# BenCooper305/RL-Cattle-Herding

Hardware: AMD Instinct MI355X
Metric: env-steps/sec (agent-steps/sec) at 4096 envs/GPU, 1/2/4/8 MI355X (higher is better)
Workload: dtype f64; 1 GPU; BASELINE configs[3]: 4096 envs/GPU x (4 drones, 16 cattle), CTDE obs (12,86), random-action rollout with auto-reset; envs_per_gpu=4096, num_drones=4, num_cattle=16, mode=ctde, physics=pyb, parallelism=env-sharded x1 (no per-step collective)

## Files before the change

### rl-cattle-herding_amd/csrc/ch_step_body.h

```cpp
#pragma once
#include <hip/hip_runtime.h>

#include <atomic>

#include "ch_common.h"
#include "ch_device.h"
#include "ch_internal.h"

namespace ch {

enum { I_N = 0, I_SC, I_SCA, I_HASPREV, I_LEVEL, I_TALLY, I_SPAWN, I_ACTIVE, I_EPISODE, I_FLOCK, I_RESET, I_NEWN,
       I_HERD, I_OBSD, I_COUNT };
static_assert(I_COUNT == kV2EnvInts, "LDS env-int rows");
enum { F_D = 0, F_T, F_H, F_A, F_E, F_R, F_X0, F_X1, F_X2,
       C_PAIRS, C_ROWS, C_COWS, C_FLOCK, C_DELTA, F_W, F_Q,
       Q_LEN, C_QUEUE, F_C,
       C_EULER,
       V_DSIMD,
       F_RSV0, F_RSV1, F_RSV2,
       F_HC,
       FLAG_COUNT };
static_assert(FLAG_COUNT <= kV2Flags, "LDS flag words");
#define FL_LIST (I_COUNT * G)
#define RS_LIST (I_COUNT * G + G)
// ... 60 lines not shown
__device__ __forceinline__ void lds_wait(int* f, int target, int* err) {
    int spins = 0;
    while (__hip_atomic_load(f, __ATOMIC_RELAXED, __HIP_MEMORY_SCOPE_WORKGROUP) < target && ++spins < (1 << 22))
        __builtin_amdgcn_s_sleep(1);
    if (spins >= (1 << 22)) handoff_failed(err);
    spin_note(spins);
    __builtin_amdgcn_fence(__ATOMIC_ACQUIRE, "workgroup", "local");
}

__device__ __forceinline__ int grab(int* ctr, int n, bool skip = false) {
    if (skip) return 1 << 28;
    int b = 0;
    if ((threadIdx.x & 63) == 0) b = atomicAdd(ctr, n);
    return __builtin_amdgcn_readfirstlane(b);
}

__device__ __forceinline__ void cow_sync(int* f, int waves, bool global, int* err) {
    if (global) __builtin_amdgcn_fence(__ATOMIC_RELEASE, "workgroup");
    lds_signal(f);
    lds_wait(f, waves, err);
    if (global) __builtin_amdgcn_fence(__ATOMIC_ACQUIRE, "workgroup");
}

#define TS(slot, val) do { if (p.tstamp) p.tstamp[(long long)blockIdx.x * 128 + (slot)] = (val); } while (0)
#define CHUNK_T0 const long long ck0_ = p.tstamp ? (long long)clock64() : 0
#define TS_MAX(slot) do { if (p.tstamp && (threadIdx.x & 63) == 0) atomicMax(reinterpret_cast<unsigned long long*>(p.tstamp + (long long)blockIdx.x * 128 + (slot)), (unsigned long long)clock64()); } while (0)
#define CHUNK_T1(loop) do { if (p.tstamp && (threadIdx.x & 63) == 0 && (threadIdx.x >> 6) <= 6) { long long* q_ = p.tstamp + (long long)blockIdx.x * 128 + 64 + 10 * ((threadIdx.x >> 6) - 1) + 2 * (loop); q_[0] += 1; q_[1] += (long long)clock64() - ck0_; } } while (0)

template <class R>
struct V2Smem {
    R *cx, *cy, *cvx, *cvy, *aux, *auy;
    R *spx, *spy;
    R *dx, *dy, *dz;
    R *pa, *pb, *sa, *sb, *ca, *cb, *scat, *psp;
    R* mrew;
    R *mq, *meor;
    R* dq;
    R *rdx, *rdy, *rdz;
    R* dcow;
    R *prev, *clock, *hcx, *hcy;
    double *dxd, *dyd, *cxd, *cyd, *hcxd, *hcyd, *prevd;
    R *tgx, *tgy, *tcx, *tcy;
    R* td;
    int* cnt;
    double* met;
    int* ei;
    int* flags;
    Level* LT;
    const uint16_t* pl;
    uint8_t *dflags, *herded, *md1, *md2;
// ... 453 lines not shown
    if (nv) { nv[u] = vx; nv[GM + u] = vy; return; }
    const long long ci = (long long)e0 * M + u;
    CH_STS(&p.cattle[2 * CS + ci], vx); CH_STS(&p.cattle[3 * CS + ci], vy);
}

template <class R>
__device__ __forceinline__ void flock_combine(const StepParams<R>& p, V2Smem<R>& S, int N, int M, int e0, int u, int n,
                                              const R* td, const uint8_t* tdf, int ib, int T) {
    const R C2B = R(2 * 4.47213595499958);
    R ddx = 0, ddy = 0, sx = 0, sy = 0, gx = 0, gy = 0, cxx = 0, cyy = 0;
    int nb = 0;
    CH_UNROLL for (int k = 0; k < N; ++k) {
        if (k >= n) break;
        const int i = ib + k;
        const int f = tdf[i];
        if (f & 1) { ++nb; gx += td[i]; gy += td[T + i]; cxx += td[2 * T + i]; cyy += td[3 * T + i]; }
        if (f & 2) { sx += td[4 * T + i]; sy += td[5 * T + i]; }
    }
    if (nb > 0) { ddx = C2B * gx + C2B * cxx; ddy = C2B * gy + C2B * cyy; }
    ddx += sx; ddy += sy;
    velocity_update(p, S, M, e0, u, ddx, ddy);
}

template <class R, int MODE, int GT, int NT, int MT, bool PHYS, bool PW, bool TOBS>
__device__ __forceinline__ void step2_body(const StepParams<R>& p, int salt = 0) {
    extern __shared__ __align__(16) unsigned char smem_[];
    unsigned char* const smem = smem_ + salt;
    constexpr bool marl = MODE == 1;
    constexpr bool MIX = sizeof(R) == 4;
    using PT = double;
    constexpr bool QUAD = !marl && GT == 16 && NT == 4;
    const int G = GT ? GT : p.G, N = NT ? NT : p.NC, M = MT ? MT : p.M, P = MT ? MT * (MT - 1) / 2 : p.P;
    const int rows = marl ? N : 12;
    const V2Layout L(G, N, M, P, MODE, (int)sizeof(R), PW ? (int)(blockDim.x >> 6) - 1 : 0, !PW && p.sep);
    const bool sep = L.sep;
    V2Smem<R> S(smem, L);
    const int BS = blockDim.x + salt, tid = threadIdx.x + salt;
    const int e0 = (blockIdx.x + salt) * G;
    const int Gv = min(G, p.E - e0);
    const long long E = p.E, DS = E * N, CS = E * M;
    const int m_obs = M < 16 ? M : 16, cat_off = marl ? 18 : 34, RW = rows * 86;
    const bool task = !(p.phase_mask & 4);
    const int W1 = (BS >> 6) - 1;
    const int ct = tid - 64, CW = BS - 64;
    int* ei = S.ei;
    int* fl = S.flags;
    const Level* LT = S.LT;
    if (tid == 0) { TS(0, (long long)wall_clock64()); TS(2, (long long)clock64()); TS(12, (long long)__smid()); }
    if ((tid & 63) == 0 && tid < 256) TS(22 + (tid >> 6), (long long)__builtin_amdgcn_s_getreg((31 << 11) | 4));

    const int nd = Gv * N;
    const bool dlane = tid < nd;
    const int dg = dlane ? tid / N : 0, dk = tid - dg * N;
    const long long di = (long long)e0 * N + tid;
    R pos[3], q[4], v[3], w[3], pid[9], ql[4], rpy_in[3] = {0, 0, 0};
    R ph_lr[4] = {0, 0, 0, 0}, ph_rr[3] = {0, 0, 0};
    int stepi = 0, n0 = 0, act0 = 0, stepi_env = 0;
    double ev_acc = 0;
    R spx_r[3] = {0, 0, 0}, spy_r[3] = {0, 0, 0};
    bool co_simd = false;
    uint8_t stale_d = 1;
    R c0[4];
    double c0d[2], prev0d;
    int ei0[10];
    R er0[2];
    double met0[kMetricRows];
    double pd[3] = {0, 0, 0};
    uint8_t stale_o = 0;
    unsigned long long tag_o = 0;
    if (tid >= 64) {
        if (ct < Gv * M) {
            const long long ci = (long long)e0 * M + ct;
#pragma unroll
            for (int c = 0; c < 4; ++c) c0[c] = p.cattle[c * CS + ci];
            if constexpr (MIX) { c0d[0] = p.cpos64[ci]; c0d[1] = p.cpos64[CS + ci]; }
        }
        if (ct < Gv) {
            const int e = e0 + ct;
#pragma unroll
            for (int r = 0; r < 9; ++r) ei0[r] = p.envi[r * E + e];
            stale_o = p.stale[E + e];
            tag_o = p.obs_tag[e];
            er0[0] = p.envr[e]; er0[1] = p.envr[E + e];
            if constexpr (MIX) prev0d = p.prev64[e];
#pragma unroll
            for (int r = 0; r < kMetricRows; ++r) met0[r] = p.metrics[r * E + e];
        }
    } else if (dlane) {
        n0 = p.envi[0 * E + e0 + dg];
        stale_d = p.stale[e0 + dg];
        if (marl) act0 = p.envi[7 * E + e0 + dg];
        pos[0] = p.drone[0 * DS + di]; pos[1] = p.drone[1 * DS + di]; pos[2] = p.drone[2 * DS + di];
        if constexpr (MIX) {
#pragma unroll
            for (int c = 0; c < 3; ++c) { pd[c] = p.pos64[c * DS + di]; pos[c] = R(pd[c]); }
        }
#pragma unroll
        for (int c = 0; c < 4; ++c) q[c] = p.drone[(3 + c) * DS + di];
#pragma unroll
        for (int c = 0; c < 3; ++c) { v[c] = p.drone[(7 + c) * DS + di]; w[c] = p.drone[(10 + c) * DS + di]; }
#pragma unroll
        for (int c = 0; c < 9; ++c) pid[c] = p.drone[(13 + c) * DS + di];
#pragma unroll
        for (int c = 0; c < 4; ++c) ql[c] = p.drone[(22 + c) * DS + di];
#pragma unroll
        for (int c = 0; c < 3; ++c) rpy_in[c] = p.rpy[c * DS + di];
        stepi = p.envi[9 * E + e0 + dg];
        if (p.evald) ev_acc = p.evald[di];
        if constexpr (PHYS) {
#pragma unroll
            for (int c = 0; c < 4; ++c) ph_lr[c] = p.phys[c * DS + di];
#pragma unroll
            for (int c = 0; c < 3; ++c) ph_rr[c] = p.phys[(4 + c) * DS + di];
        }
    }
    if (tid < Gv) stepi_env = p.envi[9 * E + e0 + tid];
    if (tid < kV2Flags) fl[tid] = 0;
    if constexpr (PW) { if (tid < G) reinterpret_cast<int*>(S.hasnb)[tid] = 0; }
    lds_barrier();

    if (tid < 64) {
        __builtin_amdgcn_s_setprio(3);
        if (tid == 0)
            __hip_atomic_store(fl + V_DSIMD, 1 + (int)((__builtin_amdgcn_s_getreg((31 << 11) | 4) >> 4) & 3), __ATOMIC_RELAXED,
                               __HIP_MEMORY_SCOPE_WORKGROUP);
    } else {
        const float rM0 = 1.0f / (float)M;
        for (int u = ct; u < Gv * M; u += CW) {
            const long long ci = (long long)e0 * M + u;
            const bool first = u == ct;
            R x = first ? c0[0] : p.cattle[0 * CS + ci], y = first ? c0[1] : p.cattle[1 * CS + ci];
            const R vx = first ? c0[2] : p.cattle[2 * CS + ci], vy = first ? c0[3] : p.cattle[3 * CS + ci];
            const R dt = R(p.dt);
            double xd = 0, yd = 0;
            if constexpr (MIX) { xd = first ? c0d[0] : p.cpos64[ci]; yd = first ? c0d[1] : p.cpos64[CS + ci]; }
            if (!PHYS || (p.physics != CH_PHYS_DYN && p.physics != CH_PHYS_DYN_RK4))
                for (int s = 0; s < p.substeps; ++s) {
                    if constexpr (MIX) { xd += (double)(vx * dt); yd += (double)(vy * dt); }
                    else { x += vx * dt; y += vy * dt; }
                }
            if constexpr (MIX) {
                x = R(xd); y = R(yd);
                CH_STS(&p.cpos64[ci], xd); CH_STS(&p.cpos64[CS + ci], yd);
                S.cxd[u] = xd; S.cyd[u] = yd;
            }
            CH_STS(&p.cattle[0 * CS + ci], x); CH_STS(&p.cattle[1 * CS + ci], y);
// ... 12 lines not shown
        const int g = ct;
        bool flk = false;
        if (g < Gv) {
            const int scA = ei0[2] + 1;
            flk = (scA % 2) == 0 && !(p.phase_mask & 2);
            ei[I_N * G + g] = ei0[0]; ei[I_SC * G + g] = ei0[1]; ei[I_SCA * G + g] = scA;
            ei[I_HASPREV * G + g] = ei0[3]; ei[I_LEVEL * G + g] = ei0[4];
            ei[I_TALLY * G + g] = ei0[5]; ei[I_SPAWN * G + g] = ei0[6];
            ei[I_ACTIVE * G + g] = ei0[7]; ei[I_EPISODE * G + g] = ei0[8];
            ei[I_FLOCK * G + g] = flk; ei[I_RESET * G + g] = 0; ei[I_HERD * G + g] = 0;
            ei0[9] = stale_o | (tag_o != (unsigned long long)(uintptr_t)p.obs ? 1 : 0);
            ei[I_OBSD * G + g] = ei0[9];
            S.prev[g] = er0[0]; S.clock[g] = er0[1];
            if constexpr (MIX) S.prevd[g] = prev0d;
#pragma unroll
            for (int r = 0; r < kMetricRows; ++r) S.met[r * G + g] = met0[r];
        }
        const unsigned long long bal = __ballot(flk);
        if (flk) ei[FL_LIST + __popcll(bal & ((1ull << ct) - 1ull))] = g;
        if (ct == 0) { ei[NF_AT] = __popcll(bal); ei[NR_AT] = 0; }
        }
        cow_sync(fl + F_E, W1, false, p.err);
        {
            int ds = lds_peek(fl + V_DSIMD);
            int spins = 0;
            for (; ds == 0 && spins < (1 << 22); ++spins) {
                __builtin_amdgcn_s_sleep(1);
                ds = lds_peek(fl + V_DSIMD);
            }
            spin_note(spins);
            co_simd = (int)((__builtin_amdgcn_s_getreg((31 << 11) | 4) >> 4) & 3) + 1 == ds;
        }
        if (ct == 0) TS(11, (long long)clock64());
        if (ct < 64) {
            const int g = ct;
            if (g < Gv) {
                PT sx = 0, sy = 0;
                CH_UNROLL for (int j = 0; j < M; ++j) { sx += S.cxd[g * M + j]; sy += S.cyd[g * M + j]; }
                S.hcxd[g] = sx / PT(M); S.hcyd[g] = sy / PT(M);
                if constexpr (MIX) { S.hcx[g] = R(S.hcxd[g]); S.hcy[g] = R(S.hcyd[g]); }
            }
            lds_signal(fl + F_HC);
        }
#pragma unroll
        for (int k = 0; k < 3; ++k) {
            const int u = ct + k * CW;
            if (u < Gv * M) {
                const int g = qdiv(u, M, rM0), j = u - g * M;
                int sp = ei[I_SPAWN * G + g] + 1;
                if (sp >= p.n_scen) sp = 0;
                const double* tab = p.spawn + ((long long)sp * p.n_cows + j) * 2;
                spx_r[k] = R(tab[0]); spy_r[k] = R(tab[1]);
            }
        }
    }
    if (tid == 0) TS(3, (long long)clock64());

    const bool wobs = !(p.phase_mask & 8);
    const bool late = sep && GT == 16 && NT == 4, fast = late && (TOBS || !p.terminal_obs);
    const bool tobs = TOBS && p.terminal_obs != nullptr;
    float* obs_wg = p.obs + (long long)e0 * RW;
    int f_n = 0, f_sc = 0, f_scA = 0, f_hp = 0, f_level = 0, f_tally = 0, f_spawn = 0, f_active = 0, f_episode = 0;
    PT f_prev = 0;
    R f_clock = 0;

    if (tid < 64) {
        const int n = dlane ? n0 : 0;
        const bool live = dlane && dk < n;
        R px0 = 0, py0 = 0;
        if (live) {
            px0 = pos[0]; py0 = pos[1];
            const int e = e0 + dg;
            float a[4];
            if (p.flags & CH_STEP_RANDOM_ACTIONS) {
                uint32_t c4[4] = {(uint32_t)stepi, 0u, (uint32_t)dk, (uint32_t)(p.env_off + e)};
                philox(c4, p.k0, p.k1);
#pragma unroll
                for (int k = 0; k < 4; ++k) a[k] = (float)(c4[k] >> 8) * (1.0f / 16777216.0f) * 2.0f - 1.0f;
                if (p.actions_out) reinterpret_cast<float4*>(p.actions_out)[di] = make_float4(a[0], a[1], a[2], a[3]);
            } else {
                float4 a4 = reinterpret_cast<const float4*>(p.actions)[di];
                a[0] = a4.x; a[1] = a4.y; a[2] = a4.z; a[3] = a4.w;
            }
            if (marl && !((act0 >> dk) & 1)) { a[0] = a[1] = a[2] = a[3] = 0.0f; }
            R Rm[9], rpy[3];
            quat_to_mat(q, Rm);
            if (stale_d == 0) { rpy[0] = rpy_in[0]; rpy[1] = rpy_in[1]; rpy[2] = rpy_in[2]; }
            else quat_to_euler(q, rpy);
            if (!(p.phase_mask & 1)) {
// ... 18 lines not shown
            if constexpr (MIX) {
#pragma unroll
                for (int c = 0; c < 3; ++c) CH_STS(&p.pos64[c * DS + di], pd[c]);
                S.dxd[tid] = pd[0]; S.dyd[tid] = pd[1];
            }
#pragma unroll
            for (int c = 0; c < 3; ++c) CH_STS(&D[c * DS + di], pos[c]);
#pragma unroll
            for (int c = 0; c < 4; ++c) CH_STS(&D[(3 + c) * DS + di], q[c]);
#pragma unroll
            for (int c = 0; c < 3; ++c) { CH_STS(&D[(7 + c) * DS + di], v[c]); CH_STS(&D[(10 + c) * DS + di], w[c]); }
#pragma unroll
            for (int c = 0; c < 9; ++c) CH_STS(&D[(13 + c) * DS + di], pid[c]);
            if (p.link_lag) {
#pragma unroll
                for (int c = 0; c < 4; ++c) CH_STS(&D[(22 + c) * DS + di], ql[c]);
            }
            S.dx[tid] = pos[0]; S.dy[tid] = pos[1]; S.dz[tid] = pos[2];
#pragma unroll
            for (int c = 0; c < 4; ++c) S.dq[c * (G * N) + tid] = q[c];
        }
        wave_sync();
        lds_signal(fl + F_D);
        if (live && wobs) obs_own_nrpy(obs_wg + dg * RW, dk, pos[2], v, w);
        if (tid == 0) TS(4, (long long)clock64());
        lds_wait(fl + F_E, W1, p.err);
        if (p.evald && live) CH_STS(&p.evald[di], eval_distance_step(ev_acc, ei[I_SC * G + dg] == 0, px0, py0, pos[0], pos[1]));

        int nb1 = -1, nb2 = -1;
        R q_pa = 0, q_pb = 0, q_sa = 0, q_sb = 0, q_ca = 0, q_cb = 0, q_ps = 0, q_sc = 0;
        int q_df = 0;
        if (live && task) {
            const int i = dk, b0 = dg * N;
            const R xi = pos[0], yi = pos[1];
            R m1 = R(INFINITY), m2 = R(INFINITY), b1 = 0, b2 = 0;
            int i1 = -1, i2 = -1;
            uint8_t f = 0;
            bool iso = true;
            CH_UNROLL for (int j = 0; j < N; ++j) {
                const bool v = j < n && j != i;
                const R d = norm2(S.dx[b0 + j] - xi, S.dy[b0 + j] - yi);
                f |= (v && d != d) ? 8 : 0;
                const bool lt1 = v && d < m1, lt2 = v && !(d < m1) && d < m2;
                m2 = lt1 ? m1 : (lt2 ? d : m2);
                m1 = lt1 ? d : m1;
                f |= (v && d < R(kCollision)) ? 2 : 0;
                iso = iso && !(v && !(d > R(kMaxFormation)));
                const bool n1 = v && (i1 < 0 || d < b1), n2 = v && !n1 && (i2 < 0 || d < b2);
                i2 = n1 ? i1 : (n2 ? j : i2);
                b2 = n1 ? b1 : (n2 ? d : b2);
                i1 = n1 ? j : i1;
                b1 = n1 ? d : b1;
            }
            if (iso) f |= 4;
            if (fabs(pos[2] - R(kTargetAlt)) > R(kTargetAlt * 0.6)) f |= 1;
            if constexpr (QUAD) {
                q_pa = m1; q_pb = m2; q_df = f;
                spacing_terms_r(LT[ei[I_LEVEL * G + dg]], p.compat != 0, m1, m2, q_sa, q_sb, q_ca, q_cb, q_ps);
            } else {
                S.pa[tid] = m1; S.pb[tid] = m2; S.dflags[tid] = f;
                spacing_terms(S, LT[ei[I_LEVEL * G + dg]], p.compat != 0, tid, m1, m2);
            }
            if (wobs) obs_nbr(obs_wg + dg * RW, S.dxd, S.dyd, b0, i, i1, i2);
            nb1 = i1; nb2 = i2;
        }
        lds_signal(fl + F_T);
        if (tid == 0) TS(5, (long long)clock64());
        const int force = (p.phase_mask & CH_PHASE_FORCE_TIMEOUT) ? 1 : 0;
        lds_wait(fl + F_HC, 1, p.err);
        const int g = QUAD ? dg : tid;
        const bool envl = QUAD ? dlane : g < Gv;
        const bool envw = envl && (!QUAD || dk == 0);
        lds_wait(fl + F_H, Gv * M + force, p.err);
        if (tid == 0) TS(6, (long long)clock64());
        if (live && task) {
            if constexpr (QUAD) q_sc = cattle_term(S, tid, M, R(p.cs_cc));
            else S.scat[tid] = cattle_term(S, tid, M, R(p.cs_cc));
            if constexpr (marl) {
                const int g = dg, n = n0, b0 = dg * N;
                const int lv = ei[I_LEVEL * G + g];
                const Level& Lv = LT[lv];
                const R a = S.pa[tid], b = S.pb[tid], sa = S.sa[tid], sb = S.sb[tid], ca = S.ca[tid], cb = S.cb[tid];
                R simple = (sa + sb) / R(2), cplx = (ca + cb) / R(2);
                if (!p.compat) {
                    if (!(b < R(INFINITY))) { simple = sa; cplx = ca; }
                    if (!(a < R(INFINITY))) { simple = 0; cplx = 0; }
                }
                R P = 0;
                P += simple * R(Lv.w_simple);
                P += cplx * R(Lv.w_complex);
                P += R(0.1) * R(Lv.w_survival);
                PT sdx = 0, sdy = 0;
                CH_UNROLL for (int i = 0; i < N; ++i) {
                    const bool li = i < n;
                    sdx += li ? S.dxd[b0 + i] : PT(0); sdy += li ? S.dyd[b0 + i] : PT(0);
                }
                sdx = divc(sdx, PT(n)); sdy = divc(sdy, PT(n));
// ... 242 lines not shown
                            }
                            CH_ST(&p.reward[(long long)e * N + i], (float)rr);
                            p.term[(long long)e * N + i] = tt;
                            p.trunc[(long long)e * N + i] = trr;
                            if (i < n && rr == rr) ret += (double)rr;
                            n_term += tt; n_trunc += trr;
                            if (i < n && (((act0 >> i) & 1) || tt) && rr != rr) n_nan += 1;
                        }
                    }
                }
            }
            rs = done && (p.flags & CH_STEP_AUTORESET);
        }
        if (envw) ei[I_RESET * G + g] = rs;
        int n_next = 0;
        if (envl && rs) n_next = p.reset_n ? p.reset_n[e] : reset_draw_n(p, f_episode, p.env_off + e);
        if (envw && rs) ei[I_NEWN * G + g] = n_next;
        const unsigned long long rbal = __ballot(envw && rs != 0);
        if (envw && rs) ei[RS_LIST + __popcll(rbal & ((1ull << tid) - 1ull))] = g;
        if (tid == 0) ei[NR_AT] = __popcll(rbal);
        if (tid == 0) TS(27, (long long)clock64());
        __builtin_amdgcn_fence(__ATOMIC_RELEASE, "workgroup");
        lds_signal(fl + F_R);
        if (tid == 0) TS(15, (long long)clock64());
        if (fast && ei[NR_AT]) {
            wave_sync();
            const bool rd = dlane && ei[I_RESET * G + dg];
            const int n_new = rd ? ei[I_NEWN * G + dg] : 0;
            if (tobs && wobs && rd && live) {
                float* tb = p.terminal_obs + (long long)(e0 + dg) * RW;
                obs_own_nrpy(tb, dk, pos[2], v, w);
                if (task) obs_nbr(tb, S.dxd, S.dyd, dg * N, dk, nb1, nb2);
            }
            double xd = 0, yd = 0, zd = 0;
            if (rd) {
                reset_drone_xyz(dk, n_new, xd, yd, zd);
                S.rdx[tid] = R(xd); S.rdy[tid] = R(yd); S.rdz[tid] = R(zd);
            }
            const R z = R(zd);
            wave_sync();
            if (rd) {
                reset_drone_store(p, di, xd, yd, zd);
                if constexpr (PHYS) {
#pragma unroll
                    for (int c = 0; c < kPhysComps; ++c) CH_STS(&p.phys[c * DS + di], R(0));
                }
                CH_STS(&p.rpy[di], R(0)); CH_STS(&p.rpy[DS + di], -R(0)); CH_STS(&p.rpy[2 * DS + di], R(0));
                if (wobs) {
                    float* eb = obs_wg + dg * RW;
                    if (dk < n_new) {
                        const R zero3[3] = {0, 0, 0}, rpy0[3] = {R(0), -R(0), R(0)};
                        obs_own(eb, dk, z, rpy0, zero3, zero3);
                        const int nb = nearest_two(S.rdx, S.rdy, dg * N, dk, n_new);
                        obs_nbr(eb, S.rdx, S.rdy, dg * N, dk, (nb & 0xff) - 1, (nb >> 8) - 1);
                    } else if (dk < ei[I_N * G + dg]) {
                        for (int c = 0; c < 14; c += 2) st2(eb, dk * 86 + c, 0.0f, 0.0f);
                    }
                }
            }
        }
        if (envl && task) {
            const int n = f_n;
            if constexpr (!marl) {
                const Level& Lv = LT[level_r];
                R sp_simple = 0, sp_complex = 0, msp = 0, mcat = 0, cat = 0;
                R psp_i[NT ? NT : 12], scat_i[NT ? NT : 12];
                CH_UNROLL for (int i = 0; i < N; ++i) {
                    const bool li = i < n;
                    const int iq = i % NQ;
                    const R pa = QUAD ? qpa[iq] : S.pa[b0 + i], pb = QUAD ? qpb[iq] : S.pb[b0 + i];
                    const bool ua = li && (p.compat || pa < R(INFINITY)), ub = li && (p.compat || pb < R(INFINITY));
                    sp_complex += ua ? (QUAD ? qca[iq] : S.ca[b0 + i]) : R(0);
                    sp_simple += ua ? (QUAD ? qsa[iq] : S.sa[b0 + i]) : R(0);
                    sp_complex += ub ? (QUAD ? qcb[iq] : S.cb[b0 + i]) : R(0);
                    sp_simple += ub ? (QUAD ? qsb[iq] : S.sb[b0 + i]) : R(0);
                    psp_i[i] = QUAD ? qps[iq] : S.psp[b0 + i]; scat_i[i] = QUAD ? qsc[iq] : S.scat[b0 + i];
                }
                const R n2 = R(n * 2.0), nn = R(n);
                sp_complex = divc(sp_complex, n2); sp_simple = divc(sp_simple, n2);
                R approach = 0;
                if (f_hp) approach = R(clip(divc(f_prev - cent, max_step_p + PT(1e-6)) * PT(5), PT(-1.0), PT(1.0)));
                f_prev = cent; f_hp = 1;
// ... 40 lines not shown
#pragma unroll
            for (int r = 0; r < kMetricRows; ++r)
                if (envw) CH_STS(&p.metrics[r * E + e], o[r]);
            if (g == 0) TS(28, (long long)clock64());
            if (p.reset_happened && envw) p.reset_happened[e] = rs;
            if (rs) reset_scalars(p, e, f_n, f_sc, f_scA, f_spawn, f_episode, f_active, f_hp, f_prev, f_clock, n_next);
            if (p.agent_active && envw)
                for (int i = 0; i < N; ++i) p.agent_active[(long long)e * N + i] = (f_active >> i) & 1;
        } else if (envw && p.reset_happened) {
            p.reset_happened[e] = 0;
        }
        if (tid == 0) TS(7, (long long)clock64());
        if (QUAD ? envw : tid < Gv) {
            const int e = e0 + (QUAD ? dg : tid);
            CH_STS(&p.envi[0 * E + e], f_n); CH_STS(&p.envi[1 * E + e], f_sc); CH_STS(&p.envi[2 * E + e], f_scA);
            CH_STS(&p.envi[3 * E + e], f_hp); CH_STS(&p.envi[4 * E + e], f_level); CH_STS(&p.envi[5 * E + e], f_tally);
            CH_STS(&p.envi[6 * E + e], f_spawn); CH_STS(&p.envi[7 * E + e], f_active); CH_STS(&p.envi[8 * E + e], f_episode);
            CH_STS(&p.envi[9 * E + e], (QUAD ? stepi : stepi_env) + 1);
            CH_STS(&p.envr[0 * E + e], R(f_prev)); CH_STS(&p.envr[1 * E + e], f_clock);
            if constexpr (MIX) CH_STS(&p.prev64[e], f_prev);
            p.stale[e] = 0;
            if (wobs) p.stale[E + e] = 0;
            p.obs_tag[e] = wobs ? (unsigned long long)(uintptr_t)p.obs : 0ull;
        }
    } else {
        const float rM = 1.0f / (float)M;
        const int nf = ei[NF_AT];
        const int* flist = ei + FL_LIST;
        const int lane = tid & 63;
        const bool co = co_simd && W1 >= 4;
        const bool skip_pre = co && (PW ? (p.phase_mask & 256) != 0 : !(p.phase_mask & 256));
        const bool skip_post = co && (p.phase_mask & 128);
        bool skip_now = skip_pre;
        R* tb = nullptr;
        uint8_t* tf = nullptr;
        uint16_t* qu = nullptr;
        int f_cur = -1, ch = 0, qn = 0, qd = 0;
        const int NCH = (P + 63) >> 6;
        constexpr int NCHC = MT > 0 ? (MT * (MT - 1) / 2 + 63) / 64 : 1;
        uint32_t prw[NCHC];
#pragma unroll
        for (int c = 0; c < NCHC; ++c) {
            const int r = 64 * c + (tid & 63);
            prw[c] = (PW && MT > 0) ? S.pl[r < P ? r : 0] : 0u;
        }
        R* const nv = S.td + 2 * G * M;
// ... 82 lines not shown
                if (p.obs_full || ei[I_OBSD * G + g]) obs_zero_env(obs_wg + g * RW, ei[I_N * G + g], rows, cat_off, m_obs, ct, CW);
        if constexpr (PW) {
            while (lds_peek(fl + F_D) < 1 && alpha_step()) {
            }
        } else {
            lds_signal(fl + F_A);
            int sleeps = 0;
            for (int spins = 0; spins < (1 << 22); ++spins) {
                if (lds_peek(fl + F_D) >= 1) break;
                if (lds_peek(fl + F_A) < W1) { __builtin_amdgcn_s_sleep(1); ++sleeps; continue; }
                __builtin_amdgcn_fence(__ATOMIC_ACQUIRE, "workgroup", "local");
                const int b = grab(fl + C_ROWS, 64, skip_pre), u = b + lane;
                if (b >= nf * M) break;
                CHUNK_T0;
                if (u < nf * M) {
                    const int f = qdiv(u, M, rM), g = flist[f], j = u - f * M;
                    alpha_row(S, M, P, g * M + j, g, j);
                    if (sep) arrive(g * M + j);
                }
                CHUNK_T1(2);
            }
            spin_note(sleeps);
        }
        if (ct == 0) TS(8, (long long)clock64());
        lds_wait(fl + F_D, 1, p.err);
        if (ct == 0) TS(9, (long long)clock64());
        skip_now = skip_post;
        for (;;) {
            const int b = grab(fl + C_COWS, 64, skip_post), u = b + lane;
            if (b >= Gv * M) break;
            CHUNK_T0;
            if (u < Gv * M) {
            const int g = qdiv(u, M, rM), j = u - g * M;
            const int n = ei[I_N * G + g], b0 = g * N;
            const R qix = S.cx[u], qiy = S.cy[u];
            CH_UNROLL for (int k = 0; k < N; ++k) {
                if (k >= n) break;
                const R ex = S.dx[b0 + k] - qix, ey = S.dy[b0 + k] - qiy;
                S.dcow[(b0 + k) * M + j] = ex * ex + ey * ey;
            }
            if (task) {
                int wn = 0;
                CH_UNROLL for (int i = 0; i < N; ++i) {
                    if (i >= n) break;
                    int i2 = (i + 1 == n) ? 0 : i + 1;
                    R x1 = S.dx[b0 + i], y1 = S.dy[b0 + i], x2 = S.dx[b0 + i2], y2 = S.dy[b0 + i2];
                    R il = (x2 - x1) * (qiy - y1) - (qix - x1) * (y2 - y1);
                    if (y1 <= qiy) { if (y2 > qiy && il > R(0)) wn += 1; }
                    else { if (y2 <= qiy && il < R(0)) wn -= 1; }
// ... 119 lines not shown
                    if (valid && k == 0) flock_combine(p, S, N, M, e0, g * M + j, n, S.td, S.tdf, (g * M + j) * N, T);
                }
                CHUNK_T1(3);
            }
            if (ct == 0) TS(16, (long long)clock64());
            if (!fuse) {
                cow_sync(fl + F_Q, W1, false, p.err);
                if (ct == 0) TS(17, (long long)clock64());
                for (;;) {
                    const int b = grab(fl + C_FLOCK, 64, skip_post), u = b + lane;
                    if (b >= nf * M) break;
                    CHUNK_T0;
                    if (u < nf * M) {
                        const int f = qdiv(u, M, rM), g = flist[f], j = u - f * M;
                        flock_combine(p, S, N, M, e0, g * M + j, ei[I_N * G + g], S.td, S.tdf, (g * M + j) * N, T);
                    }
                    CHUNK_T1(4);
                }
            }
            }
        }
        if (lane == 0) TS(40 + (tid >> 6), (long long)clock64());
        TS_MAX(57);
        if (ct == 0) TS(31, (long long)nf);
        lds_wait(fl + F_R, 1, p.err);
        if (tid == 64) TS(37, (long long)clock64());
        const int nr = ei[NR_AT];
        if (ct == 0) TS(30, (long long)nr);
        if (nr && ct == 0) TS(52, (long long)clock64());
        TS_MAX(56);
        if (late) {
            const bool ew = Gv * M > CW - 64 || ct - lane >= Gv * M;
            if (ew) euler_pass();
            TS_MAX(58);
            for (int u = ct; u < Gv * M; u += CW) {
                const int g = qdiv(u, M, rM), j = u - g * M;
                const bool rs_ = fast && ei[I_RESET * G + g];
                const int n_old = ei[I_N * G + g];
                const long long ci = (long long)e0 * M + u;
                if (rs_) {
                    if (tobs && wobs && j < m_obs)
                        obs_cattle(p.terminal_obs + (long long)(e0 + g) * RW, S.dxd, S.dyd, g * N, j, n_old, cat_off,
                                   S.cxd[u], S.cyd[u]);
                    const double x = MIX ? spawn_d(g, j, 0) : (double)S.spx[u], y = MIX ? spawn_d(g, j, 1) : (double)S.spy[u];
                    p.cattle[0 * CS + ci] = R(x); p.cattle[1 * CS + ci] = R(y);
                    if constexpr (MIX) { p.cpos64[ci] = x; p.cpos64[CS + ci] = y; }
                    if (!ei[I_FLOCK * G + g]) {
                        R vx, vy;
                        reset_cow_vel(p, ci, p.env_off + e0 + g, j, (uint32_t)ei[I_EPISODE * G + g], vx, vy);
// ... 77 lines not shown
                        obs_own(eb, k, R(rz), rpy0, zero3, zero3);
                        const int nb = nearest_two(S.rdx, S.rdy, g * N, k, n);
                        obs_nbr(eb, S.rdx, S.rdy, g * N, k, (nb & 0xff) - 1, (nb >> 8) - 1);
                    } else if (k < ei[I_N * G + g]) {
                        for (int c = 0; c < 86; c += 2) st2(eb, k * 86 + c, 0.0f, 0.0f);
                    }
                }
            }
            if (ct >= c0l)
                for (int u = ct - c0l, i = 0; u < nr * M; u += cl, ++i) {
                    const int k0 = qdiv(u, M, rM), g = rl[k0], j = u - k0 * M, uc = g * M + j;
                    R vx = i == 0 ? cvx_r[0] : cvx_r[1], vy = i == 0 ? cvy_r[0] : cvy_r[1];
                    if (i >= RI)
                        reset_cow_vel(p, (long long)e0 * M + uc, p.env_off + e0 + g, j, (uint32_t)ei[I_EPISODE * G + g], vx, vy);
                    const double x = MIX ? spawn_d(g, j, 0) : (double)S.spx[uc], y = MIX ? spawn_d(g, j, 1) : (double)S.spy[uc];
                    reset_cow_store(p, (long long)e0 * M + uc, x, y, vx, vy);
                    if (wobs && j < m_obs) obs_cattle(obs_wg + g * RW, S.rdx, S.rdy, g * N, j, ei[I_NEWN * G + g], cat_off, x, y);
                }
            if (ct == 0) TS(54, (long long)clock64());
        }
    }
    if (tid == 0) TS(35, (long long)clock64());
    if (tid == 64) TS(36, (long long)clock64());
    if (tid >= 64) TS_MAX(63);
    if (p.tstamp) {
        lds_barrier();
        if (tid == 0) { TS(13, (long long)clock64()); TS(14, (long long)clock64()); TS(1, (long long)wall_clock64()); }
    }
}

}
```

### rl-cattle-herding_amd/csrc/ch_step_multi.hip

```cpp
#include "ch_step_body.h"

namespace ch {

template <class R, int MODE, int GT, int NT, int MT, bool PHYS, bool PW>
__device__ __forceinline__ void step2_once(const StepParams<R>* p, int salt) {
    const unsigned long long a = (unsigned long long)(uintptr_t)p;
    const unsigned lo = __builtin_amdgcn_readfirstlane((unsigned)a), hi = __builtin_amdgcn_readfirstlane((unsigned)(a >> 32));
    using KP = const __attribute__((address_space(4))) StepParams<R>*;
    const KP kp = (KP)(((unsigned long long)hi << 32) | lo);
    step2_body<R, MODE, GT, NT, MT, PHYS, PW, false>(*(const StepParams<R>*)kp, salt);
}
#ifndef CH_MULTI_MAX_BLOCK
#define CH_MULTI_MAX_BLOCK CH_V2_MAX_BLOCK_PW
#endif
template <class R, int MODE, int GT, int NT, int MT, bool PHYS = false, bool PW = false, int WPE = 1>
__global__ __launch_bounds__(PW ? CH_V2_MAX_BLOCK_PW : CH_MULTI_MAX_BLOCK)
__attribute__((amdgpu_waves_per_eu(WPE)))
void k_step2_multi(const StepParams<R>* __restrict__ pd, int n_steps) {
    for (int k = 0; k < n_steps; ++k) {
        int salt = 0;
        const StepParams<R>* q = pd;
        asm volatile("" : "+s"(salt), "+s"(q));
        step2_once<R, MODE, GT, NT, MT, PHYS, PW>(q, salt);
        __builtin_amdgcn_fence(__ATOMIC_RELEASE, "workgroup");
        __builtin_amdgcn_s_barrier();
        __builtin_amdgcn_fence(__ATOMIC_ACQUIRE, "workgroup");
        __builtin_amdgcn_s_setprio(0);
    }
}

template <class R, int MODE, int GT, int NT, int MT, bool PHYS = false, bool PW = false, int WPE = 1>
static hipError_t launch_v2_multi_kernel(const StepParams<R>& p, const StepParams<R>* pd, int block, size_t lds,
                                         hipStream_t st, int n_steps, bool launch) {
    static std::atomic<unsigned long long> attr_set{0};
    int dev = 0;
    hipError_t e = hipGetDevice(&dev);
    if (e != hipSuccess) return e;
    const unsigned long long bit = 1ull << (dev & 63);
    if (!(attr_set.load(std::memory_order_relaxed) & bit)) {
        e = hipFuncSetAttribute(reinterpret_cast<const void*>(&k_step2_multi<R, MODE, GT, NT, MT, PHYS, PW, WPE>),
                                hipFuncAttributeMaxDynamicSharedMemorySize, 160 * 1024);
        if (e != hipSuccess) return e;
        attr_set.fetch_or(bit, std::memory_order_relaxed);
    }
    if (!launch) return hipSuccess;
    dim3 grid((p.E + p.G - 1) / p.G);
    hipLaunchKernelGGL((k_step2_multi<R, MODE, GT, NT, MT, PHYS, PW, WPE>), grid, dim3(block < (PW ? CH_V2_MAX_BLOCK_PW : CH_MULTI_MAX_BLOCK) ? block : (PW ? CH_V2_MAX_BLOCK_PW : CH_MULTI_MAX_BLOCK)),
                       lds, st, pd, n_steps);
    return hipGetLastError();
}

template <class R>
hipError_t launch_step_v2_multi(const StepParams<R>& p, const StepParams<R>* pd, int block, size_t lds, hipStream_t st,
                                int n_steps, bool launch) {
    const int G = p.G, N = p.NC, M = p.M;
    if (p.physics != CH_PHYS_PYB || p.terminal_obs) return hipErrorNotSupported;
    if constexpr (sizeof(R) == sizeof(double)) {
        if (p.pw) {
            if (p.mode == 1 && G == 16 && N == 4 && M == 32)
                return launch_v2_multi_kernel<R, 1, 16, 4, 32, false, true>(p, pd, block, lds, st, n_steps, launch);
            return hipErrorNotSupported;
        }
        if (p.mode != 0) return hipErrorNotSupported;
        if (G == 16 && N == 4 && M == 16) return launch_v2_multi_kernel<R, 0, 16, 4, 16>(p, pd, block, lds, st, n_steps, launch);
        if (G == 8 && N == 4 && M == 16) return launch_v2_multi_kernel<R, 0, 8, 4, 16>(p, pd, block, lds, st, n_steps, launch);
        if (G == 16 && N == 2 && M == 8) return launch_v2_multi_kernel<R, 0, 16, 2, 8>(p, pd, block, lds, st, n_steps, launch);
// ... 24 lines not shown
```

Baseline: 275.0 million env-steps/s.

## Pipeline consecutive env steps across two drone waves in the multi-step kernel

For the f64 (16 envs, 4 drones, 16 cattle) multi-step kernel, two drone waves now alternate steps. Drone state is handed between them through LDS and the per-step flag and position buffers are double-buffered, so step k+1's drone physics can start while the cattle waves are still finishing step k. The block-wide barrier between steps is replaced with LDS counter signals (P_N, P_B, P_C). This adds LDS usage and more complex synchronisation, and launch now fails with not-supported when the block size, separate-layout flag or LDS budget do not fit.

```diff
diff --git a/rl-cattle-herding_amd/csrc/ch_step_body.h b/rl-cattle-herding_amd/csrc/ch_step_body.h
--- a/rl-cattle-herding_amd/csrc/ch_step_body.h
+++ b/rl-cattle-herding_amd/csrc/ch_step_body.h
@@ -106,10 +106,13 @@
     if (global) __builtin_amdgcn_fence(__ATOMIC_ACQUIRE, "workgroup");
 }
 
-#define TS(slot, val) do { if (p.tstamp) p.tstamp[(long long)blockIdx.x * 128 + (slot)] = (val); } while (0)
-#define CHUNK_T0 const long long ck0_ = p.tstamp ? (long long)clock64() : 0
-#define TS_MAX(slot) do { if (p.tstamp && (threadIdx.x & 63) == 0) atomicMax(reinterpret_cast<unsigned long long*>(p.tstamp + (long long)blockIdx.x * 128 + (slot)), (unsigned long long)clock64()); } while (0)
-#define CHUNK_T1(loop) do { if (p.tstamp && (threadIdx.x & 63) == 0 && (threadIdx.x >> 6) <= 6) { long long* q_ = p.tstamp + (long long)blockIdx.x * 128 + 64 + 10 * ((threadIdx.x >> 6) - 1) + 2 * (loop); q_[0] += 1; q_[1] += (long long)clock64() - ck0_; } } while (0)
+#define TS(slot, val) do { if (!PIPE && p.tstamp) p.tstamp[(long long)blockIdx.x * 128 + (slot)] = (val); } while (0)
+#define CHUNK_T0 const long long ck0_ = (!PIPE && p.tstamp) ? (long long)clock64() : 0
+#define TS_MAX(slot) do { if (!PIPE && p.tstamp && (threadIdx.x & 63) == 0) atomicMax(reinterpret_cast<unsigned long long*>(p.tstamp + (long long)blockIdx.x * 128 + (slot)), (unsigned long long)clock64()); } while (0)
+#define CHUNK_T1(loop) do { if (!PIPE && p.tstamp && (threadIdx.x & 63) == 0 && (threadIdx.x >> 6) <= 6) { long long* q_ = p.tstamp + (long long)blockIdx.x * 128 + 64 + 10 * ((threadIdx.x >> 6) - 1) + 2 * (loop); q_[0] += 1; q_[1] += (long long)clock64() - ck0_; } } while (0)
+
+#define PTS(i, val) do { if (PIPE && p.tstamp && kstep < 8) p.tstamp[(long long)blockIdx.x * 128 + 16 * kstep + (i)] = (val); } while (0)
+#define PTS_MAX(i) do { if (PIPE && p.tstamp && kstep < 8 && (threadIdx.x & 63) == 0) atomicMax(reinterpret_cast<unsigned long long*>(p.tstamp + (long long)blockIdx.x * 128 + 16 * kstep + (i)), (unsigned long long)clock64()); } while (0)
 
 template <class R>
 struct V2Smem {
@@ -609,10 +612,25 @@
     velocity_update(p, S, M, e0, u, ddx, ddy);
 }
 
-template <class R, int MODE, int GT, int NT, int MT, bool PHYS, bool PW, bool TOBS>
-__device__ __forceinline__ void step2_body(const StepParams<R>& p, int salt = 0) {
+template <class R>
+struct V2Pipe {
+    enum { P_N = 0, P_B, P_C, P_SIMD, P_COUNT = 8 };
+    static constexpr size_t kBytes = (27 + 7) * 64 * sizeof(R) + (2 * 64 + kV2Flags + P_COUNT) * sizeof(int);
+    R *ho, *d1;
+    int *hoi, *flags1, *sync;
+    __device__ explicit V2Pipe(unsigned char* base) {
+        ho = (R*)base; d1 = ho + 27 * 64;
+        hoi = (int*)(d1 + 7 * 64); flags1 = hoi + 2 * 64; sync = flags1 + kV2Flags;
+    }
+};
+
+template <class R, int MODE, int GT, int NT, int MT, bool PHYS, bool PW, bool TOBS, int ROLE = 0>
+__device__ __forceinline__ void step2_body(const StepParams<R>& p, int salt = 0, int kstep = 0) {
     extern __shared__ __align__(16) unsigned char smem_[];
     unsigned char* const smem = smem_ + salt;
+    constexpr bool PIPE = ROLE != 0;
+    static_assert(!PIPE || (sizeof(R) == 8 && MODE == 0 && GT == 16 && NT == 4 && !PW && !TOBS && !PHYS),
+                  "the pipelined step loop is the configs[3] f64 instantiation's");
     constexpr bool marl = MODE == 1;
     constexpr bool MIX = sizeof(R) == 4;
     using PT = double;
@@ -622,7 +640,19 @@
     const V2Layout L(G, N, M, P, MODE, (int)sizeof(R), PW ? (int)(blockDim.x >> 6) - 1 : 0, !PW && p.sep);
     const bool sep = L.sep;
     V2Smem<R> S(smem, L);
-    const int BS = blockDim.x + salt, tid = threadIdx.x + salt;
+    const int BS = (PIPE ? (int)blockDim.x - 64 : (int)blockDim.x) + salt;
+    const int tid = (ROLE == 1 ? (int)(threadIdx.x & 63) : ROLE == 2 ? (int)threadIdx.x - 64 : (int)threadIdx.x) + salt;
+    const bool isd = ROLE == 1 ? true : ROLE == 2 ? false : tid < 64;
+    const V2Pipe<R> X(smem + (PIPE ? L.bytes() : 0));
+    int* const ps = X.sync;
+    int* const flags0 = S.flags;
+    if constexpr (PIPE) {
+        if (kstep & 1) {
+            S.dx = X.d1; S.dy = S.dx + G * N; S.dz = S.dy + G * N; S.dq = S.dz + G * N;
+            S.dxd = (double*)S.dx; S.dyd = (double*)S.dy;
+            S.flags = X.flags1;
+        }
+    }
     const int e0 = (blockIdx.x + salt) * G;
     const int Gv = min(G, p.E - e0);
     const long long E = p.E, DS = E * N, CS = E * M;
@@ -634,7 +664,7 @@
     int* fl = S.flags;
     const Level* LT = S.LT;
     if (tid == 0) { TS(0, (long long)wall_clock64()); TS(2, (long long)clock64()); TS(12, (long long)__smid()); }
-    if ((tid & 63) == 0 && tid < 256) TS(22 + (tid >> 6), (long long)__builtin_amdgcn_s_getreg((31 << 11) | 4));
+    if ((tid & 63) == 0 && tid < 256 && !PIPE) TS(22 + (tid >> 6), (long long)__builtin_amdgcn_s_getreg((31 << 11) | 4));
 
     const int nd = Gv * N;
     const bool dlane = tid < nd;
@@ -655,7 +685,26 @@
     double pd[3] = {0, 0, 0};
     uint8_t stale_o = 0;
     unsigned long long tag_o = 0;
-    if (tid >= 64) {
+    if constexpr (PIPE) {
+        if (ROLE == 1 && tid == 0) { PTS(0, (long long)clock64()); PTS(7, (long long)__builtin_amdgcn_s_getreg((31 << 11) | 4)); }
+        if (ROLE == 2 && ct == 0) PTS(8, (long long)clock64());
+        if (kstep > 0) {
+            if (ROLE == 2) {
+                lds_wait(ps + V2Pipe<R>::P_B, kstep, p.err);
+                __builtin_amdgcn_fence(__ATOMIC_RELEASE, "workgroup");
+                lds_signal(ps + V2Pipe<R>::P_C);
+                lds_wait(ps + V2Pipe<R>::P_C, W1 * kstep, p.err);
+                __builtin_amdgcn_fence(__ATOMIC_ACQUIRE, "workgroup");
+                int* const flp = (kstep & 1) ? flags0 : X.flags1;
+                if (ct < kV2Flags) flp[ct] = 0;
+            } else {
+                lds_wait(ps + V2Pipe<R>::P_N, kstep, p.err);
+            }
+        }
+        if (ROLE == 1 && tid == 0) PTS(1, (long long)clock64());
+        if (ROLE == 2 && ct == 0) PTS(9, (long long)clock64());
+    }
+    if (!isd) {
         if (ct < Gv * M) {
             const long long ci = (long long)e0 * M + ct;
 #pragma unroll
@@ -673,6 +722,20 @@
 #pragma unroll
             for (int r = 0; r < kMetricRows; ++r) met0[r] = p.metrics[r * E + e];
         }
+    } else if (PIPE && kstep > 0) {
+        const R* ho = X.ho + tid;
+        pos[0] = ho[0 * 64]; pos[1] = ho[1 * 64]; pos[2] = ho[2 * 64];
+#pragma unroll
+        for (int c = 0; c < 4; ++c) q[c] = ho[(3 + c) * 64];
+#pragma unroll
+        for (int c = 0; c < 3; ++c) { v[c] = ho[(7 + c) * 64]; w[c] = ho[(10 + c) * 64]; }
+#pragma unroll
+        for (int c = 0; c < 9; ++c) pid[c] = ho[(13 + c) * 64];
+#pragma unroll
+        for (int c = 0; c < 4; ++c) ql[c] = ho[(22 + c) * 64];
+        ev_acc = ho[26 * 64];
+        n0 = X.hoi[tid]; stepi = X.hoi[64 + tid];
+        stale_d = 1;
     } else if (dlane) {
         n0 = p.envi[0 * E + e0 + dg];
         stale_d = p.stale[e0 + dg];
@@ -701,14 +764,16 @@
             for (int c = 0; c < 3; ++c) ph_rr[c] = p.phys[(4 + c) * DS + di];
         }
     }
+    if constexpr (!PIPE) {
     if (tid < Gv) stepi_env = p.envi[9 * E + e0 + tid];
     if (tid < kV2Flags) fl[tid] = 0;
     if constexpr (PW) { if (tid < G) reinterpret_cast<int*>(S.hasnb)[tid] = 0; }
     lds_barrier();
-
-    if (tid < 64) {
+    }
+
+    if (isd) {
         __builtin_amdgcn_s_setprio(3);
-        if (tid == 0)
+        if (tid == 0 && !PIPE)
             __hip_atomic_store(fl + V_DSIMD, 1 + (int)((__builtin_amdgcn_s_getreg((31 << 11) | 4) >> 4) & 3), __ATOMIC_RELAXED,
                                __HIP_MEMORY_SCOPE_WORKGROUP);
     } else {
@@ -767,9 +832,9 @@
         }
         cow_sync(fl + F_E, W1, false, p.err);
         {
-            int ds = lds_peek(fl + V_DSIMD);
+            int ds = PIPE ? ps[V2Pipe<R>::P_SIMD + (kstep & 1)] : lds_peek(fl + V_DSIMD);
             int spins = 0;
-            for (; ds == 0 && spins < (1 << 22); ++spins) {
+            for (; ds == 0 && spins < (1 << 22) && !PIPE; ++spins) {
                 __builtin_amdgcn_s_sleep(1);
                 ds = lds_peek(fl + V_DSIMD);
             }
@@ -809,7 +874,7 @@
     PT f_prev = 0;
     R f_clock = 0;
 
-    if (tid < 64) {
+    if (isd) {
         const int n = dlane ? n0 : 0;
         const bool live = dlane && dk < n;
         R px0 = 0, py0 = 0;
@@ -874,10 +939,29 @@
         }
         wave_sync();
         lds_signal(fl + F_D);
+        if constexpr (PIPE) {
+            R* ho = X.ho + tid;
+            ho[0 * 64] = pos[0]; ho[1 * 64] = pos[1]; ho[2 * 64] = pos[2];
+#pragma unroll
+            for (int c = 0; c < 4; ++c) ho[(3 + c) * 64] = q[c];
+#pragma unroll
+            for (int c = 0; c < 3; ++c) { ho[(7 + c) * 64] = v[c]; ho[(10 + c) * 64] = w[c]; }
+#pragma unroll
+            for (int c = 0; c < 9; ++c) ho[(13 + c) * 64] = pid[c];
+#pragma unroll
+            for (int c = 0; c < 4; ++c) ho[(22 + c) * 64] = ql[c];
+            X.hoi[tid] = n0; X.hoi[64 + tid] = stepi + 1;
+        }
         if (live && wobs) obs_own_nrpy(obs_wg + dg * RW, dk, pos[2], v, w);
-        if (tid == 0) TS(4, (long long)clock64());
+        if (tid == 0) { TS(4, (long long)clock64()); PTS(2, (long long)clock64()); }
+        if constexpr (PIPE) __builtin_amdgcn_s_setprio(0);
         lds_wait(fl + F_E, W1, p.err);
-        if (p.evald && live) CH_STS(&p.evald[di], eval_distance_step(ev_acc, ei[I_SC * G + dg] == 0, px0, py0, pos[0], pos[1]));
+        if constexpr (PIPE) __builtin_amdgcn_s_setprio(3);
+        if (p.evald && live) {
+            ev_acc = eval_distance_step(ev_acc, ei[I_SC * G + dg] == 0, px0, py0, pos[0], pos[1]);
+            CH_STS(&p.evald[di], ev_acc);
+        }
+        if constexpr (PIPE) X.ho[26 * 64 + tid] = ev_acc;
 
         int nb1 = -1, nb2 = -1;
         R q_pa = 0, q_pb = 0, q_sa = 0, q_sb = 0, q_ca = 0, q_cb = 0, q_ps = 0, q_sc = 0;
@@ -924,7 +1008,7 @@
         const bool envl = QUAD ? dlane : g < Gv;
         const bool envw = envl && (!QUAD || dk == 0);
         lds_wait(fl + F_H, Gv * M + force, p.err);
-        if (tid == 0) TS(6, (long long)clock64());
+        if (tid == 0) { TS(6, (long long)clock64()); PTS(3, (long long)clock64()); }
         if (live && task) {
             if constexpr (QUAD) q_sc = cattle_term(S, tid, M, R(p.cs_cc));
             else S.scat[tid] = cattle_term(S, tid, M, R(p.cs_cc));
@@ -1213,7 +1297,7 @@
         if (tid == 0) TS(27, (long long)clock64());
         __builtin_amdgcn_fence(__ATOMIC_RELEASE, "workgroup");
         lds_signal(fl + F_R);
-        if (tid == 0) TS(15, (long long)clock64());
+        if (tid == 0) { TS(15, (long long)clock64()); PTS(4, (long long)clock64()); }
         if (fast && ei[NR_AT]) {
             wave_sync();
             const bool rd = dlane && ei[I_RESET * G + dg];
@@ -1231,6 +1315,20 @@
             const R z = R(zd);
             wave_sync();
             if (rd) {
+                if constexpr (PIPE) {
+                    R* ho = X.ho + tid;
+                    ho[0 * 64] = R(xd); ho[1 * 64] = R(yd); ho[2 * 64] = R(zd);
+                    ho[3 * 64] = 0; ho[4 * 64] = 0; ho[5 * 64] = 0; ho[6 * 64] = 1;
+#pragma unroll
+                    for (int c = 7; c < 13; ++c) ho[c * 64] = 0;
+                    if (!p.compat) {
+#pragma unroll
+                        for (int c = 13; c < 22; ++c) ho[c * 64] = 0;
+                    }
+                    ho[22 * 64] = 0; ho[23 * 64] = 0; ho[24 * 64] = 0; ho[25 * 64] = 1;
+                    ho[26 * 64] = 0;
+                    X.hoi[tid] = n_new;
+                }
                 reset_drone_store(p, di, xd, yd, zd);
                 if constexpr (PHYS) {
 #pragma unroll
@@ -1249,6 +1347,11 @@
                     }
                 }
             }
+        }
+        if constexpr (PIPE) {
+            __builtin_amdgcn_fence(__ATOMIC_RELEASE, "workgroup");
+            lds_signal(ps + V2Pipe<R>::P_N);
+            if (tid == 0) PTS(5, (long long)clock64());
         }
         if (envl && task) {
             const int n = f_n;
@@ -1335,6 +1438,11 @@
             p.stale[e] = 0;
             if (wobs) p.stale[E + e] = 0;
             p.obs_tag[e] = wobs ? (unsigned long long)(uintptr_t)p.obs : 0ull;
+        }
+        if constexpr (PIPE) {
+            __builtin_amdgcn_fence(__ATOMIC_RELEASE, "workgroup");
+            lds_signal(ps + V2Pipe<R>::P_B);
+            if (tid == 0) PTS(6, (long long)clock64());
         }
     } else {
         const float rM = 1.0f / (float)M;
@@ -1463,9 +1571,9 @@
             }
             spin_note(sleeps);
         }
-        if (ct == 0) TS(8, (long long)clock64());
+        if (ct == 0) { TS(8, (long long)clock64()); PTS(10, (long long)clock64()); }
         lds_wait(fl + F_D, 1, p.err);
-        if (ct == 0) TS(9, (long long)clock64());
+        if (ct == 0) { TS(9, (long long)clock64()); PTS(11, (long long)clock64()); }
         skip_now = skip_post;
         for (;;) {
             const int b = grab(fl + C_COWS, 64, skip_post), u = b + lane;
@@ -1631,9 +1739,10 @@
         }
         if (lane == 0) TS(40 + (tid >> 6), (long long)clock64());
         TS_MAX(57);
-        if (ct == 0) TS(31, (long long)nf);
+        if (ct == 0) { TS(31, (long long)nf); PTS(12, (long long)clock64()); }
+        PTS_MAX(13);
         lds_wait(fl + F_R, 1, p.err);
-        if (tid == 64) TS(37, (long long)clock64());
+        if (tid == 64) { TS(37, (long long)clock64()); PTS(14, (long long)clock64()); }
         const int nr = ei[NR_AT];
         if (ct == 0) TS(30, (long long)nr);
         if (nr && ct == 0) TS(52, (long long)clock64());
@@ -1757,11 +1866,26 @@
     }
     if (tid == 0) TS(35, (long long)clock64());
     if (tid == 64) TS(36, (long long)clock64());
-    if (tid >= 64) TS_MAX(63);
+    if (tid >= 64) { TS_MAX(63); PTS_MAX(15); }
     if (p.tstamp) {
-        lds_barrier();
+        if constexpr (!PIPE) lds_barrier();
         if (tid == 0) { TS(13, (long long)clock64()); TS(14, (long long)clock64()); TS(1, (long long)wall_clock64()); }
     }
 }
 
-}
+
+template <class R, int MODE, int GT, int NT, int MT>
+__device__ __forceinline__ void step2_pipe_init(const StepParams<R>& p) {
+    extern __shared__ __align__(16) unsigned char smem_[];
+    const V2Layout L(GT, NT, MT, MT * (MT - 1) / 2, MODE, (int)sizeof(R), 0, p.sep != 0);
+    V2Smem<R> S(smem_, L);
+    const V2Pipe<R> X(smem_ + L.bytes());
+    const int t = threadIdx.x;
+    if (t < kV2Flags) { S.flags[t] = 0; X.flags1[t] = 0; }
+    if (t < V2Pipe<R>::P_SIMD) X.sync[t] = 0;
+    if ((t & 63) == 0 && t < 128)
+        X.sync[V2Pipe<R>::P_SIMD + (t >> 6)] = 1 + (int)((__builtin_amdgcn_s_getreg((31 << 11) | 4) >> 4) & 3);
+    lds_barrier();
+}
+
+}
diff --git a/rl-cattle-herding_amd/csrc/ch_step_multi.hip b/rl-cattle-herding_amd/csrc/ch_step_multi.hip
--- a/rl-cattle-herding_amd/csrc/ch_step_multi.hip
+++ b/rl-cattle-herding_amd/csrc/ch_step_multi.hip
@@ -2,14 +2,21 @@
 
 namespace ch {
 
-template <class R, int MODE, int GT, int NT, int MT, bool PHYS, bool PW>
-__device__ __forceinline__ void step2_once(const StepParams<R>* p, int salt) {
+template <class R>
+__device__ __forceinline__ const StepParams<R>& uniform_params(const StepParams<R>* p) {
     const unsigned long long a = (unsigned long long)(uintptr_t)p;
     const unsigned lo = __builtin_amdgcn_readfirstlane((unsigned)a), hi = __builtin_amdgcn_readfirstlane((unsigned)(a >> 32));
     using KP = const __attribute__((address_space(4))) StepParams<R>*;
     const KP kp = (KP)(((unsigned long long)hi << 32) | lo);
-    step2_body<R, MODE, GT, NT, MT, PHYS, PW, false>(*(const StepParams<R>*)kp, salt);
+    return *(const StepParams<R>*)kp;
 }
+template <class R, int MODE, int GT, int NT, int MT, bool PHYS, bool PW, int ROLE = 0>
+__device__ __forceinline__ void step2_once(const StepParams<R>* p, int salt, int kstep = 0) {
+    step2_body<R, MODE, GT, NT, MT, PHYS, PW, false, ROLE>(uniform_params(p), salt, kstep);
+}
+
+template <class R, int MODE, int GT, int NT, int MT, bool PHYS, bool PW, int WPE>
+constexpr bool kMultiPipelined = sizeof(R) == 8 && MODE == 0 && GT == 16 && NT == 4 && MT == 16 && !PHYS && !PW && WPE == 1;
 #ifndef CH_MULTI_MAX_BLOCK
 #define CH_MULTI_MAX_BLOCK CH_V2_MAX_BLOCK_PW
 #endif
@@ -17,6 +24,26 @@
 __global__ __launch_bounds__(PW ? CH_V2_MAX_BLOCK_PW : CH_MULTI_MAX_BLOCK)
 __attribute__((amdgpu_waves_per_eu(WPE)))
 void k_step2_multi(const StepParams<R>* __restrict__ pd, int n_steps) {
+    if constexpr (kMultiPipelined<R, MODE, GT, NT, MT, PHYS, PW, WPE>) {
+        step2_pipe_init<R, MODE, GT, NT, MT>(uniform_params(pd));
+        const int wave = __builtin_amdgcn_readfirstlane((int)(threadIdx.x >> 6));
+        if (wave < 2) {
+            for (int k = wave; k < n_steps; k += 2) {
+                int salt = 0;
+                const StepParams<R>* q = pd;
+                asm volatile("" : "+s"(salt), "+s"(q));
+                step2_once<R, MODE, GT, NT, MT, PHYS, PW, 1>(q, salt, k);
+                __builtin_amdgcn_s_setprio(0);
+            }
+        } else {
+            for (int k = 0; k < n_steps; ++k) {
+                int salt = 0;
+                const StepParams<R>* q = pd;
+                asm volatile("" : "+s"(salt), "+s"(q));
+                step2_once<R, MODE, GT, NT, MT, PHYS, PW, 2>(q, salt, k);
+            }
+        }
+    } else {
     for (int k = 0; k < n_steps; ++k) {
         int salt = 0;
         const StepParams<R>* q = pd;
@@ -26,6 +53,7 @@
         __builtin_amdgcn_s_barrier();
         __builtin_amdgcn_fence(__ATOMIC_ACQUIRE, "workgroup");
         __builtin_amdgcn_s_setprio(0);
+    }
     }
 }
 
@@ -42,6 +70,12 @@
                                 hipFuncAttributeMaxDynamicSharedMemorySize, 160 * 1024);
         if (e != hipSuccess) return e;
         attr_set.fetch_or(bit, std::memory_order_relaxed);
+    }
+    if constexpr (kMultiPipelined<R, MODE, GT, NT, MT, PHYS, PW, WPE>) {
+        const int blk = block < CH_MULTI_MAX_BLOCK ? block : CH_MULTI_MAX_BLOCK;
+        if (blk < 256 || p.G * p.M > 3 * (blk - 128) || !p.sep || lds + V2Pipe<R>::kBytes > 160 * 1024)
+            return hipErrorNotSupported;
+        lds += V2Pipe<R>::kBytes;
     }
     if (!launch) return hipSuccess;
     dim3 grid((p.E + p.G - 1) / p.G);
```

Result: faster. 292.2 million env-steps/s (median of 6 runs) (+6.2%).
